# amoretti86/phylo

Measured on AMD Instinct MI355X. Metric: particle-site-likelihoods/sec, higher is better.
Workload: dtype f64; 1 GPU; primate.p N=12 S=898, GTR-init (jcmodel=false), K=2048 per GPU (K_total=2048), lambda=10, full sweep of 11 rank events; parallelism=particles sharded over 1 GPU(s), global resampling, sweeps_per_launch_set=16, contexts_in_flight=3, sweeps_in_flight=48, particles_in_flight=98304

## Files before the change

include/phylo_hip.h:

```cpp
#ifndef PHYLO_HIP_H
#define PHYLO_HIP_H

#include <stdint.h>

#ifdef __cplusplus
extern "C" {
#endif

typedef struct phylo_ctx phylo_ctx;

enum {
    PHYLO_OK = 0,
    PHYLO_EINVAL = -1,
    PHYLO_ENODEVICE = -2,
    PHYLO_EHIP = -3,
    PHYLO_ENOMEM = -4,
    PHYLO_ECOMM = -5,
    PHYLO_ESTATE = -6
};

enum {
    PHYLO_QUIRK_Q1_RAW_Q = 1u << 0,
    PHYLO_TWISTING = 1u << 1,
    PHYLO_TIME_KERNELS = 1u << 2,
// ... 91 lines not shown

int phylo_debug_stamps(phylo_ctx* ctx, uint64_t* out, int n);

int phylo_debug_reverse_lists(int N, int K, const int64_t* ancestors, const int32_t* child, int early_free, int rows_form,
                              const int32_t* lookahead_nodes, int n_lookahead, int32_t* lists, int64_t n_lists, int32_t* meta,
                              int n_meta);

int phylo_debug_lookahead_lists(int N, int K, int S, int M, const int32_t* roots_ad, int32_t* slow_flag, int32_t* image,
                                int64_t n_image, int32_t* meta, int n_meta);

int phylo_debug_reverse_plan(int N, int K, int K_local, int S, int world, int twisted, int marks, uint32_t switches, int64_t n_slow,
                             int TS, int64_t coeff_wgs, int passes_in_flight, uint32_t* mask);
int phylo_debug_sweep_plan(int N, int K, int K_local, int S, int G, int M, int world, int transport, uint32_t flags, uint32_t switches,
                           uint32_t* mask, int32_t* launches);
int phylo_debug_pack_leaf_codes(const uint8_t* codes, int N, int S, uint8_t* packed, int64_t cap, int64_t* need);
int phylo_debug_reverse_plan_batch(int N, int K, int G, int S, uint32_t switches, int64_t n_slow, int TS, int64_t coeff_wgs,
                                   int passes_in_flight, uint32_t* mask);
int phylo_debug_tree_plan(int N, int K, int G, int world, int64_t n_clades, int64_t n_topologies, int kept_whole, int64_t summary_temp,
                          int64_t branches_temp, int64_t* scalars, int64_t* summary_slab, int64_t* branches_slab, int32_t* sort_bits,
                          int32_t* launches);

int phylo_debug_device_lists(phylo_ctx* ctx, int32_t* lists, int64_t n_lists, int32_t* meta, int n_meta, int64_t* ancestors,
                             int32_t* child);
int phylo_debug_device_lists_of(phylo_ctx* ctx, const int64_t* ancestors, const int32_t* child, int32_t* lists, int64_t n_lists,
                                int32_t* meta, int n_meta);

int phylo_tree_summary(phylo_ctx* ctx, int64_t* n_clades, int32_t* n_topologies, int32_t* n_groups, phylo_stats* perf);
int phylo_tree_summary_fetch(phylo_ctx* ctx, uint64_t* clade_bits, uint64_t* clade_weight, int32_t* clade_group, uint64_t* topo_weight,
                             int32_t* topo_count, int32_t* topo_rep, int32_t* topo_group, int32_t* particle_topo, uint64_t* u, uint64_t* U);

// ... 25 lines not shown
```

phylo_amd/_ffi.py:

```python
from __future__ import annotations

import ctypes as C
import os

import numpy as np

_HERE = os.path.dirname(os.path.abspath(__file__))
LIB_PATH = os.path.join(_HERE, "csrc", "libphylo_hip.so")

PHYLO_OK = 0
QUIRK_Q1_RAW_Q = 1 << 0
TWISTING = 1 << 1
TIME_KERNELS = 1 << 2
EAGER_NODES = 1 << 3
KEEP_GRAPH = 1 << 4
ONE_LAUNCH = 1 << 5
FLAGS_DEFAULT = QUIRK_Q1_RAW_Q
COMM_ID_BYTES = 128

EXPORTS = [
    "phylo_version", "phylo_last_error", "phylo_device_count", "phylo_create", "phylo_destroy",
    "phylo_set_leaves", "phylo_set_model", "phylo_expm_batched", "phylo_cond_likelihood_K",
    "phylo_forest_loglik", "phylo_tree_loglik", "phylo_trees_loglik", "phylo_trees_loglik_rates", "phylo_debug_tree_schedule", "phylo_resample", "phylo_log_zsmc", "phylo_sweep",
    "phylo_sweep_async", "phylo_sweep_batch_async", "phylo_sweep_batch_begin", "phylo_sweep_fetch_logz", "phylo_sweep_begin", "phylo_sweep_step", "phylo_sweep_step_a", "phylo_sweep_step_group", "phylo_sweep_finish", "phylo_sweep_fetch",
    "phylo_synchronize", "phylo_sweep_node", "phylo_sweep_backward", "phylo_sweep_backward_batch",
    "phylo_tree_summary", "phylo_tree_summary_fetch", "phylo_tree_branches", "phylo_tree_branches_fetch",
    "phylo_math_probe", "phylo_debug_frechet", "phylo_debug_stamps", "phylo_debug_reverse_lists", "phylo_debug_lookahead_lists", "phylo_debug_reverse_plan", "phylo_debug_reverse_plan_batch", "phylo_debug_sweep_plan", "phylo_debug_pack_leaf_codes", "phylo_debug_tree_plan", "phylo_debug_device_lists", "phylo_debug_device_lists_of", "phylo_debug_remote_cache", "phylo_debug_site_product",
    "phylo_vi_gradients", "phylo_vi_gradients_batch", "phylo_vi_apply",
    "phylo_site_tile", "phylo_set_site_tile", "phylo_get_site_tile",
    "phylo_comm_unique_id", "phylo_comm_init", "phylo_comm_share", "phylo_comm_allgather", "phylo_comm_max", "phylo_comm_barrier",
    "phylo_comm_exchange_kind",
]


class PhyloError(RuntimeError):
    def __init__(self, code, msg):
        super().__init__("libphylo_hip error %d: %s" % (code, msg))
        self.code = code


class Stats(C.Structure):
    _fields_ = [("sweep_ms", C.c_double), ("merge_ms", C.c_double), ("merge_launches", C.c_int32),
# ... 116 lines not shown
def debug_pack_leaf_codes(codes):
    lib = load()
    cd = np.ascontiguousarray(codes, dtype=np.uint8)
    if cd.ndim != 2:
        raise ValueError("codes must be [N][S]")
    N, S = cd.shape
    need = C.c_int64(0)
    rc = lib.phylo_debug_pack_leaf_codes(_ptr(cd), C.c_int(N), C.c_int(S), None, C.c_int64(0), C.byref(need))
    if rc:
        raise PhyloError(rc, lib.phylo_last_error(None).decode())
    out = np.full(need.value, 0xff, dtype=np.uint8)
    rc = lib.phylo_debug_pack_leaf_codes(_ptr(cd), C.c_int(N), C.c_int(S), _ptr(out), C.c_int64(out.size), C.byref(need))
    if rc:
        raise PhyloError(rc, lib.phylo_last_error(None).decode())
    return out.reshape(N, -1, 64, 16)


TREE_SUMMARY_BUFS = ("u", "U", "bits", "kA", "kB", "val", "scan", "weight", "srt", "hp", "o_cbits", "o_cw", "o_tw", "child", "slot", "o_cg",
                     "o_tn", "o_trep", "o_tg", "o_ptopo", "vA", "vB", "flag", "sid", "cid", "seg_start", "count", "group", "first", "tid", "pos",
                     "err", "vC", "vD", "temp")
TREE_BRANCHES_BUFS = ("ebr", "lbr", "gbl", "gbr", "o_cs", "o_ls", "o_ts", "wA", "wB", "cpos", "kA", "kB", "vA", "vB", "cstart", "toff", "o_tc",
                      "temp")


def debug_tree_plan(N, K, G=1, world=1, n_clades=1, n_topologies=1, kept_whole=False, summary_temp=0, branches_temp=0):
    lib = load()
    ns, nb = len(TREE_SUMMARY_BUFS), len(TREE_BRANCHES_BUFS)
    sc = (C.c_int64 * 13)()
    ss, bs = (C.c_int64 * (2 * ns + 1))(), (C.c_int64 * (2 * nb + 1))()
    bits, launches = (C.c_int32 * 17)(), (C.c_int32 * 2)()
# ... 454 lines not shown

    def comm_allgather_blob(self, a):
        a = np.ascontiguousarray(a)
        world = self.K // self.K_local
        if world == 1:
            return a[None]
        out = np.empty((world,) + a.shape, dtype=a.dtype)
        self._check(self._lib.phylo_comm_allgather(self._h, _ptr(a), C.c_size_t(a.nbytes), _ptr(out)))
        return out

    def debug_remote_cache(self):
        used, cap = C.c_int(0), C.c_int(0)
        self._check(self._lib.phylo_debug_remote_cache(self._h, C.byref(used), C.byref(cap)))
        return used.value, cap.value

    def comm_exchange_kind(self):
        return ('none', 'rccl', 'hostshm', 'p2p')[int(self._lib.phylo_comm_exchange_kind(self._h))]

    def comm_max(self, value):
        v = C.c_double(float(value))
        self._check(self._lib.phylo_comm_max(self._h, C.byref(v)))
        return v.value

    def comm_barrier(self):
        self._check(self._lib.phylo_comm_barrier(self._h))


def sweep_step_group(ctxs):
    arr = (C.c_void_p * len(ctxs))(*[c._h for c in ctxs])
    rc = load().phylo_sweep_step_group(arr, C.c_int(len(ctxs)))
# ... 11 lines not shown
```

phylo_amd/csrc/phylo_hip.hip:

```cpp
#include "../../include/phylo_hip.h"

#include <cstring>
#include <hip/hip_runtime.h>
#include <hip/hip_ext.h>
#include <rocprim/device/device_radix_sort.hpp>

#include <cstdarg>
#include <cstdio>
#include <cstdlib>
#include <atomic>
#include <chrono>
#include <mutex>
#include <string>
#include <vector>

#include "phylo_comm.h"
#include "phylo_kernels.h"
#include "phylo_packed_codes.h"
#include "phylo_persist.h"
#include "phylo_grad.h"
#include "phylo_revlists_dev.h"
#include "phylo_sweep_plan.h"
#include "phylo_train.h"
#include "phylo_trees.h"
#include "phylo_trees_plan.h"
#include "phylo_treeset.h"

#include <algorithm>
#include <type_traits>

namespace {

thread_local std::string g_last_error;
// ... 12 lines not shown
    bool active = false;
    int a_done_r = -1;
    sweep_plan plan{};
};

struct env_switches {
    bool eager_nodes = false, rehearse_sharded = false, replicated_book = false, no_leaf_codes = false, one_launch = false,
         persist_stamps = false, grad_one_stream = false, grad_two_streams = false, rev_host_lists = false, no_remote_cache = false,
         no_p2p = false, grad_rows_chain = false, grad_coeff_chain = false;
    int persist_wgs = 0;
    unsigned long long p2p_wait_ticks = PK_P2P_WAIT_TICKS;
    size_t p2p_copy_words = 65536;
    int persist_nt = 256;
    int remote_cache_cap = 0;
    int scan_multi_min = 4096;
    int trees_chunk = 0;
    void read() {
        eager_nodes = getenv("PHYLO_EAGER_NODES") != nullptr;
        rehearse_sharded = getenv("PHYLO_REHEARSE_SHARDED") != nullptr;
        replicated_book = getenv("PHYLO_REPLICATED_BOOK") != nullptr;
        grad_rows_chain = getenv("PHYLO_GRAD_ROWS_CHAIN") != nullptr;
        grad_coeff_chain = getenv("PHYLO_GRAD_COEFF_CHAIN") != nullptr;
        no_leaf_codes = getenv("PHYLO_NO_LEAF_CODES") != nullptr;
        one_launch = getenv("PHYLO_ONE_LAUNCH") != nullptr;
        persist_stamps = getenv("PHYLO_PERSIST_STAMPS") != nullptr;
        grad_one_stream = getenv("PHYLO_GRAD_ONE_STREAM") != nullptr;
        grad_two_streams = getenv("PHYLO_GRAD_TWO_STREAMS") != nullptr;
        rev_host_lists = getenv("PHYLO_REV_HOST_LISTS") != nullptr;
        no_remote_cache = getenv("PHYLO_NO_REMOTE_CACHE") != nullptr;
        { const char* e = getenv("PHYLO_REMOTE_CACHE_CAP"); remote_cache_cap = e ? atoi(e) : 0; }
        { const char* e = getenv("PHYLO_SCAN_MULTI_MIN"); scan_multi_min = e ? atoi(e) : 4096; }
        { const char* e = getenv("PHYLO_TREES_CHUNK"); trees_chunk = e ? atoi(e) : 0; }
        { const char* e = getenv("PHYLO_P2P"); no_p2p = e && atoi(e) == 0; }
        { const char* e = getenv("PHYLO_P2P_COPY_WORDS"); p2p_copy_words = e ? (size_t)atol(e) : 65536; }
        { const char* e = getenv("PHYLO_P2P_WAIT_S"); p2p_wait_ticks = e && atof(e) > 0 ? (unsigned long long)(atof(e) * 1e8) : PK_P2P_WAIT_TICKS; }
        const char* w = getenv("PHYLO_PERSIST_WGS");
        persist_wgs = w ? atoi(w) : 0;
        const char* t = getenv("PHYLO_PERSIST_NT");
        persist_nt = (t && atoi(t) == 512) ? 512 : 256;
    }
};

struct phylo_ctx {
    int device = 0;
    env_switches env;
// ... 9 lines not shown
    int K = 0, N = 0, S = 0, A = 4;
    int Kloc = 0, k0 = 0;
    int rank = 0, world = 1;
    uint32_t flags = 0;
    hipStream_t stream = nullptr;
    hipEvent_t ev0 = nullptr, ev1 = nullptr;
    std::vector<hipEvent_t> kev;
    std::string err;
    bool have_leaves = false, have_model = false, swept = false, state_ready = false;
    int jc = 0;
    std::vector<double> h_lam_l, h_lam_r, h_ldf;
    double *d_Q = nullptr, *d_pi = nullptr, *d_lam_l = nullptr, *d_lam_r = nullptr, *d_ldf = nullptr;
    double* d_leaves = nullptr;
    uint8_t* d_leaf_codes = nullptr;
    uint8_t* d_leaf_packed = nullptr;
    bool leaves_coded = false;
    uint32_t* d_pair_hist = nullptr;
    bool hist_ready = false, codes_valid = false;
    double* d_pool = nullptr;
    double* d_nodell = nullptr;
    double *d_bl = nullptr, *d_br = nullptr, *d_Pmat = nullptr;
    double *d_logw = nullptr, *d_ll = nullptr;
    double* d_aux = nullptr;
    unsigned long long* d_rec = nullptr;
    int tile_override = 0;
    int site_tile = 0, ntiles = 1;
    double* d_tilev = nullptr;
    double* d_lse = nullptr;
    uint64_t* d_group_seeds = nullptr;
    char* d_tables = nullptr;
// ... 543 lines not shown
    do {
        if ((rc = bind(c)) != PHYLO_OK) break;
        {
            hipDeviceProp_t prop;
            if (hipGetDeviceProperties(&prop, dev) != hipSuccess) { rc = fail(c, PHYLO_EHIP, "hipGetDeviceProperties failed"); break; }
            c->n_cus = prop.multiProcessorCount;
        }
        if (hipStreamCreateWithFlags(&c->stream, hipStreamNonBlocking) != hipSuccess) { rc = fail(c, PHYLO_EHIP, "hipStreamCreate failed"); break; }
        if (hipEventCreate(&c->ev0) != hipSuccess || hipEventCreate(&c->ev1) != hipSuccess) { rc = fail(c, PHYLO_EHIP, "hipEventCreate failed"); break; }
        if ((rc = dalloc(c, &c->d_Q, 20 + 2 * (size_t)N)) != PHYLO_OK) break;
        c->d_pi = c->d_Q + 16;
        c->d_lam_l = c->d_Q + 20;
        c->d_lam_r = c->d_Q + 20 + N;
        if ((rc = dalloc(c, &c->d_ldf, (size_t)N + 1)) != PHYLO_OK) break;
        if ((rc = dalloc(c, &c->d_leaves, (size_t)N * S * 4)) != PHYLO_OK) break;
        if ((rc = dalloc(c, &c->d_leaf_codes, pk_codes_image_bytes(N, S))) != PHYLO_OK) break;
        c->d_leaf_packed = c->d_leaf_codes + pk_packed_offset(N, S);
        c->h_ldf.resize((size_t)N + 1);
        for (int cnt = 0; cnt <= N; ++cnt) c->h_ldf[cnt] = host_log_double_factorial(2 * (cnt > 2 ? cnt : 2) - 3);
        if (hipMemcpy(c->d_ldf, c->h_ldf.data(), ((size_t)N + 1) * 8, hipMemcpyHostToDevice) != hipSuccess) { rc = fail(c, PHYLO_EHIP, "ldf upload failed"); break; }
    } while (0);
    if (rc != PHYLO_OK) {
        g_last_error = c->err;
        phylo_destroy(c);
        return rc;
    }
    *out = c;
    return PHYLO_OK;
}

int phylo_destroy(phylo_ctx* c) {
    if (!c) return PHYLO_OK;
// ... 49 lines not shown
    HIPCHK(c, hipStreamSynchronize(c->stream));
    c->tile_override = T;
    c->site_tile = T ? T : pm_site_tile(c->S);
    c->ntiles = (c->S + c->site_tile - 1) / c->site_tile;
    free_sweep_state(c);
    c->state_ready = false;
    c->swept = false; ++c->sweep_serial;
    c->ts_done = c->tb_done = false;
    return PHYLO_OK;
}

int phylo_set_leaves(phylo_ctx* c, const double* genome) {
    CHK(bind(c));
    if (!genome) return fail(c, PHYLO_EINVAL, "genome_NxSxA is NULL");
    const size_t rows = (size_t)c->N * c->S;
    const size_t code_bytes = pk_codes_image_bytes(c->N, c->S);
    const bool pinned = rows * 32 + code_bytes <= ((size_t)8 << 20);
    std::vector<uint8_t> codes_v;
    uint8_t* codes = nullptr;
    if (pinned) {
        if (!c->h_leaves_p) {
            HIPCHK(c, hipHostMalloc((void**)&c->h_leaves_p, rows * 32 + code_bytes));
            HIPCHK(c, hipEventCreateWithFlags(&c->ev_leaves, hipEventDisableTiming));
        } else {
            HIPCHK(c, hipEventSynchronize(c->ev_leaves));
        }
        memcpy(c->h_leaves_p, genome, rows * 32);
        HIPCHK(c, hipMemcpyAsync(c->d_leaves, c->h_leaves_p, rows * 32, hipMemcpyHostToDevice, c->stream));
        codes = (uint8_t*)c->h_leaves_p + rows * 32;
    } else {
        HIPCHK(c, hipMemcpyAsync(c->d_leaves, genome, rows * 32, hipMemcpyHostToDevice, c->stream));
// ... 4 lines not shown
        bool ok = true;
        for (size_t i = 0; i < rows && ok; ++i) {
            const double* x = genome + i * 4;
            int ones = 0, zeros = 0, last = 0;
            for (int j = 0; j < 4; ++j) {
                if (pm_bits(x[j]) == pm_bits(1.0)) { ++ones; last = j; }
                else if (pm_bits(x[j]) == 0) ++zeros;
            }
            if (ones == 1 && zeros == 3) codes[i] = (uint8_t)last;
            else if (ones == 4) codes[i] = 4;
            else ok = false;
        }
        c->codes_valid = ok;
        c->leaves_coded = ok && !c->env.no_leaf_codes;
        c->hist_ready = false;
        if (ok) {
            pk_pack_leaf_codes(codes, c->N, c->S, codes + pk_packed_offset(c->N, c->S));
            HIPCHK(c, hipMemcpyAsync(c->d_leaf_codes, codes, code_bytes, hipMemcpyHostToDevice, c->stream));
        }
    }
    if (pinned) HIPCHK(c, hipEventRecord(c->ev_leaves, c->stream));
    c->have_leaves = true;
    c->last_graph = c->last_graph_twist = false;
    c->leaves_newer = true;
    CHK(refresh_leaf_ll(c));
    if (!pinned) HIPCHK(c, hipStreamSynchronize(c->stream));
    return PHYLO_OK;
}

int phylo_set_model(phylo_ctx* c, const double* Q16, const double* pi4, const double* lam_l, const double* lam_r,
                    int jc69_closed_form) {
    CHK(bind(c));
    if (!Q16 || !pi4 || !lam_l || !lam_r) return fail(c, PHYLO_EINVAL, "NULL model pointer");
// ... 664 lines not shown
    a.flag_off = c->x_flag_off[purpose];
    a.epoch = ++c->x_epoch[purpose];
    a.timeout_word = c->d_counter + 1;
    a.wait_ticks = c->env.p2p_wait_ticks;
    const size_t words = (size_t)n_arrays * count * (size_t)(c->world - 1);
    if (words > c->env.p2p_copy_words) {
        const size_t wgs = (words + 4095) / 4096;
        hipLaunchKernelGGL(pk_p2p_copy, dim3((unsigned)(wgs < 512 ? wgs : 512)), dim3(1024), 0, c->stream, a);
        CHK(launch_check(c, "pk_p2p_copy"));
        a.n_seg = 0;
    }
    hipLaunchKernelGGL(pk_p2p_exchange, dim3(1), dim3(1024), 0, c->stream, a);
    return launch_check(c, "pk_p2p_exchange");
}

static pk_rank_args rank_args(const phylo_ctx* c, int r) {
    const sweep_plan& p = c->run.plan;
    const int N = c->N, K = c->K, Kl = c->Kloc, cur = r & 1, nxt = cur ^ 1;
    const size_t plane = (size_t)K * N;
    pk_rank_args b{};
    b.r = r; b.n = N - r; b.N = N; b.S = c->S; b.K = K; b.Kloc = Kl; b.k0 = c->k0;
    b.seed = c->run.seed; b.flags = c->run.flags;
    b.Kg = p.Kg; b.group_seeds = p.G > 1 ? c->d_group_seeds : nullptr;
    b.no_store = (r == p.R - 1 && p.no_store_last) ? 1 : 0;
    if (p.graph) {
        b.roots_old = c->d_hroots + plane * r; b.cnt_old = c->d_hcnt + plane * r;
        b.roots_new = c->d_hroots + plane * (r + 1); b.cnt_new = c->d_hcnt + plane * (r + 1);
        b.rootll_old = c->d_hrootll + plane * r; b.rootll_new = c->d_hrootll + plane * (r + 1);
        b.pos_hist = c->d_pos + plane * r;
    } else {
// ... 137 lines not shown
    return launch_check(c, "pk_rank_book_packed");
}

static int step_merge(phylo_ctx* c, const pk_rank_args& b) {
    const sweep_plan& p = c->run.plan;
    const int S = c->S;
    const dim3 mgrid((unsigned)((size_t)c->Kloc * c->ntiles));
    hipEvent_t e0 = nullptr, e1 = nullptr;
    if (p.timek && !p.twist) { e0 = c->kev[2 * b.r]; e1 = c->kev[2 * b.r + 1]; }
    if (!(b.lazy || b.no_store)) {
        const size_t lds = (size_t)(c->site_tile < S ? c->site_tile : S) * 8 + 16 + PK_STORE_STAGE_BYTES;
        launch_stamped(pk_rank_merge, mgrid, dim3(PK_COLS), lds, c->stream, e0, e1, b);
    } else if (b.rec) {
        pk_pi4 pi4;
        memcpy(pi4.v, c->h_model_p + 16, sizeof pi4.v);
        launch_stamped(pk_rank_merge_nostore, mgrid, dim3(64), 0, c->stream, e0, e1, (const unsigned long long*)b.rec, b.Pmat, S, b.T,
                       b.ntiles, b.tilev, pi4);
    } else {
        launch_stamped(pk_rank_merge_nostore_ids, mgrid, dim3(64), 0, c->stream, e0, e1, b);
    }
    return launch_check(c, "pk_rank_merge");
}

static int step_tiles(phylo_ctx* c, const pk_rank_args& b) {
    hipLaunchKernelGGL(pk_tile_epilogue, dim3(cdiv(c->Kloc, 256)), dim3(256), 0, c->stream, b);
    return launch_check(c, "pk_tile_epilogue");
}

static int step_exchange(phylo_ctx* c, int r) {
    const size_t K = c->K;
    double* rows[3] = {c->d_logw + r * K, c->d_ll + r * K, c->d_nodell + c->N + r * K};
    return comm_exchange(c, rows, 3, (size_t)c->Kloc, 0);
// ... 1074 lines not shown
    const sweep_plan p = sweep_plan_form(f, k_sweep_limits);
    *mask = sweep_plan_mask(p);
    for (int r = -1; r <= p.R; ++r) launches[r + 1] = sweep_plan_launches(p, r);
    return PHYLO_OK;
}

int phylo_debug_pack_leaf_codes(const uint8_t* codes, int N, int S, uint8_t* packed, int64_t cap, int64_t* need) {
    if (N < 1 || S < 1 || !need || (packed && !codes)) return fail(nullptr, PHYLO_EINVAL, "phylo_debug_pack_leaf_codes: bad arguments");
    *need = (int64_t)pk_packed_bytes(N, S);
    if (!packed) return PHYLO_OK;
    if (cap < *need) return fail(nullptr, PHYLO_EINVAL, "phylo_debug_pack_leaf_codes: the image takes %lld bytes (got %lld)", (long long)*need, (long long)cap);
    pk_pack_leaf_codes(codes, N, S, packed);
    return PHYLO_OK;
}

int phylo_debug_tree_plan(int N, int K, int G, int world, int64_t n_clades, int64_t n_topologies, int kept_whole, int64_t summary_temp,
                          int64_t branches_temp, int64_t* scalars, int64_t* summary_slab, int64_t* branches_slab, int32_t* sort_bits,
                          int32_t* launches) {
    if (K < 1 || G < 1 || K % G != 0 || N > PK_MAX_TAXA || world < 1 || summary_temp < 0 || branches_temp < 0 || !scalars || !summary_slab ||
        !branches_slab || !sort_bits || !launches)
        return fail(nullptr, PHYLO_EINVAL, "phylo_debug_tree_plan: bad arguments");
    char why[160];
    const pt_facts f{N, K, G, world};
    if (pt_refuses(f, why, sizeof why)) return fail(nullptr, PHYLO_EINVAL, "%s", why);
    const pb_facts fb{N, K, G, world, n_clades, n_topologies, kept_whole != 0};
    if (pb_refuses(fb, why, sizeof why)) return fail(nullptr, PHYLO_ESTATE, "%s", why);
    pt_plan p = pt_plan_form(f);
    pt_plan_slab(p, (size_t)summary_temp);
    pb_plan q = pb_plan_form(fb);
    pb_plan_slab(q, (size_t)branches_temp);
// ... 643 lines not shown
```

phylo_amd/csrc/phylo_kernels.h:

```cpp
#pragma once
#include <hip/hip_runtime.h>
#include <stdint.h>

#include "phylo_math.h"
#include "phylo_packed_codes.h"

#define PK_COLS 256
#define PK_AUX 8
#define PK_MAX_TAXA 512
#define PK_MAX_GROUPS 64

enum { AUX_SUM_REM = 0, AUX_FPRIOR, AUX_LPRIOR, AUX_RPRIOR, AUX_LL_TILDE, AUX_PAREN, AUX_LOGV, AUX_Q };
#define PK_REC 16
enum { REC_BASE_L = PK_AUX, REC_BASE_R, REC_NODELL, REC_ROOTLL, REC_LL, REC_LOGW, REC_FLAGS  };
#define PK_REC_SLOTS (REC_FLAGS + 1)
static_assert(PK_REC_SLOTS <= PK_REC && PK_REC_SLOTS <= 16, "one lane per slot: with 16 lanes or more per particle the bookkeeping writes the record in one trip (pk_book_tail)");

__device__ __forceinline__ double pk_block_canon_sum(double col, double* sh4) {
#pragma unroll
    for (int off = 1; off < 64; off <<= 1) col = col + __shfl_xor(col, off, 64);
    __syncthreads();
    if ((threadIdx.x & 63) == 0) sh4[threadIdx.x >> 6] = col;
    __syncthreads();
    return ((sh4[0] + sh4[1]) + sh4[2]) + sh4[3];
// ... 1568 lines not shown
            pk_rows_pair_spec<CL, CR>(A, B, cw & 0xffu, (cw >> 8) & 0xffu, s, s1, bl, br, Pl, Pr, tabL, tabR, pi, col, flag);
            lo >>= 16;
        }
        if (m & 1) {
            if ((m >> 1) == 4) lo = hi;
            (CL ? A.cl : A.cr) = (unsigned int)lo & 0xffu;
            double xa = pk_rows_lik<CL, CR>(A, Pl, Pr, tabL, tabR, nullptr, pi);
            xa = s < s1 ? xa : 1.0;
            pm_lp_mul_spec(col, xa, flag);
        }
        if (n <= 16) break;
        n -= 16; ++Jc;
    }
    return pm_lp_flag_set(flag);
}
template <bool CL, bool CR>
__device__ __forceinline__ pm_lp pk_rows_general_v(int s0, int s1, const char* bl, const char* br, const pk_cdbl* Pc, const pk_cdbl* pik,
                                                   double (*tabL)[4], double (*tabR)[4], double* lik25) {
    const double pi[4] = {pik[0], pik[1], pik[2], pik[3]};
    double Pl[16], Pr[16];
#pragma unroll
    for (int u = 0; u < 16; ++u) {
        Pl[u] = CL ? 0.0 : Pc[u];
        Pr[u] = CR ? 0.0 : Pc[16 + u];
    }
    pk_rowregs A;
    pk_cstream c;
    pm_lp col = pm_lp_init();
    pk_cs_request<CL, CR>(c, bl, br, s0 >> 10);
    pk_rows_load_u<CL, CR>(A, bl, br, s0 + (int)(threadIdx.x & 63), s1);
    pk_rows_run_packed<CL, CR>(s0, s1, bl, br, A, c, Pl, Pr, tabL, tabR, lik25, pi, col);
    return col;
}
__device__ __forceinline__ pm_lp pk_rows_general(unsigned int fl, int s0, int s1, const char* bl, const char* br, const double* Pu,
                                                 const double* pi4, double (*tabL)[4], double (*tabR)[4], double* lik25) {
    fl = (unsigned int)__builtin_amdgcn_readfirstlane((int)fl);
    s0 = __builtin_amdgcn_readfirstlane(s0);
    s1 = __builtin_amdgcn_readfirstlane(s1);
    bl = pk_uniform_ptr(bl);
    br = pk_uniform_ptr(br);
    const pk_cdbl* Pc = (const pk_cdbl*)pk_uniform_ptr(Pu);
    const pk_cdbl* pik = (const pk_cdbl*)pk_uniform_ptr(pi4);
    if ((fl & 3u) == 3u) return pk_rows_general_v<true, true>(s0, s1, bl, br, Pc, pik, tabL, tabR, lik25);
    if (fl & 1u) return pk_rows_general_v<true, false>(s0, s1, bl, br, Pc, pik, tabL, tabR, lik25);
    return pk_rows_general_v<false, true>(s0, s1, bl, br, Pc, pik, tabL, tabR, lik25);
}
template <bool CL, bool CR>
__device__ __forceinline__ bool pk_rows_loop_rec(int s0, int s1, const char* bl, const char* br, const double* Pu, const pk_cdbl* Pc,
                                                 double (*tabL)[4], double (*tabR)[4], double* lik25, const pk_cdbl* pik, pm_lp& col) {
    const int lane = threadIdx.x & 63;
    const double pi[4] = {pik[0], pik[1], pik[2], pik[3]};
    double Pl[16], Pr[16];
#pragma unroll
    for (int u = 0; u < 16; ++u) {
        Pl[u] = CL ? 0.0 : Pc[u];
        Pr[u] = CR ? 0.0 : Pc[16 + u];
    }
    if constexpr (CL != CR) {
#pragma unroll
        for (int u = 0; u < 16; ++u) asm volatile("" : "+s"(CL ? Pr[u] : Pl[u]));
    }
    pk_rowregs A;
    pk_cstream c;
    if constexpr (CL || CR) {
// ... 16 lines not shown
        pk_wave_lds_fence();
    }
    if constexpr (CL || CR) {
        if (!redo) {
            bool flag;
            if constexpr (CL && CR) flag = pk_rows_fast_cc(s0, s1, bl, br, c, lik25, col);
            else flag = pk_rows_fast_mixed<CL, CR>(s0, s1, bl, br, A, c, Pl, Pr, tabL, tabR, pi, col);
            redo = __any(flag);
        }
        return redo;
    } else {
        pk_rows_run<CL, CR>(s0, s1, bl, br, A, Pl, Pr, tabL, tabR, lik25, pi, col);
        return false;
    }
}
struct pk_merge_kernarg { const unsigned long long* rec; const double* Pmat; int S, T, ntiles; double* tilev; pk_pi4 pi4; };
__global__ __launch_bounds__(64) __attribute__((amdgpu_waves_per_eu(7, 8), amdgpu_num_vgpr(32)))
void pk_rank_merge_nostore(const unsigned long long* __restrict__ rec, const double* __restrict__ Pmat, int S, int T, int ntiles,
                           double* __restrict__ tilev, const pk_pi4 pi4) {
    __shared__ __attribute__((aligned(16))) double tabL[PK_PAD_CODE + 1][4], tabR[PK_PAD_CODE + 1][4];
    __shared__ double lik25[PK_PAD_CODE * 6 + 1];
    const int item = (int)blockIdx.x;
    const int k = __builtin_amdgcn_readfirstlane(ntiles == 1 ? item : item / ntiles), tau = item - k * ntiles;
    const int s0 = __builtin_amdgcn_readfirstlane(tau * T), s1 = __builtin_amdgcn_readfirstlane(s0 + T < S ? s0 + T : S);
    const pk_cu64* rc = (const pk_cu64*)(rec + (size_t)k * PK_REC);
    const double* Pu = Pmat + (size_t)k * 32;
    const pk_cdbl* Pc = (const pk_cdbl*)Pu;
    PK_TOUCH4_DECL;
    PK_TOUCH4_256(Pu);
    unsigned int fl = (unsigned int)rc[REC_FLAGS];
    const char* bl = pk_uniform_ptr((const void*)rc[REC_BASE_L]);
    const char* br = pk_uniform_ptr((const void*)rc[REC_BASE_R]);
    PK_TOUCH4_END(fl);
    static_assert(offsetof(pk_merge_kernarg, pi4) == 40 && sizeof(pk_merge_kernarg) == 72, "the kernel's argument segment");
    const pk_cdbl* pi = (const pk_cdbl*)((__attribute__((address_space(4))) const char*)__builtin_amdgcn_kernarg_segment_ptr() +
                                         offsetof(pk_merge_kernarg, pi4));
    pm_lp col = pm_lp_init();
    bool redo;
    if (fl & 1u) {
        if (fl & 2u) redo = pk_rows_loop_rec<true, true>(s0, s1, bl, br, Pu, Pc, tabL, tabR, lik25, pi, col);
        else redo = pk_rows_loop_rec<true, false>(s0, s1, bl, br, Pu, Pc, tabL, tabR, lik25, pi, col);
    } else {
        if (fl & 2u) redo = pk_rows_loop_rec<false, true>(s0, s1, bl, br, Pu, Pc, tabL, tabR, lik25, pi, col);
        else redo = pk_rows_loop_rec<false, false>(s0, s1, bl, br, Pu, Pc, tabL, tabR, lik25, pi, col);
    }
    if (redo) col = pk_rows_general(fl, s0, s1, bl, br, Pu, (const double*)pi, tabL, tabR, lik25);
    const double tot = pk_wave_tree_sum(pm_lp_finish(col));
    if (threadIdx.x == 0) {
        if (ntiles != 1) {
            tilev[(size_t)k * ntiles + tau] = tot;
        } else {
            const pk_cdbl* ax = (const pk_cdbl*)rc;
            const double fl2 = ax[AUX_SUM_REM] + tot;
            const double ll = ((fl2 + ax[AUX_FPRIOR]) + ax[AUX_LPRIOR]) + ax[AUX_RPRIOR];
            const double lw = (((ll - ax[AUX_LL_TILDE]) - ax[AUX_PAREN]) + ax[AUX_LOGV]) - ax[AUX_Q];
            *(pk_gd*)rc[REC_NODELL] = tot;
            *(pk_gd*)rc[REC_ROOTLL] = tot;
            *(pk_gd*)rc[REC_LL] = ll;
            *(pk_gd*)rc[REC_LOGW] = lw;
// ... 597 lines not shown
```

Before: 611.9 billion particle-site-likelihoods/s.

## Compress alignment columns into unique site patterns for the root merge kernel

```diff
diff --git a/include/phylo_hip.h b/include/phylo_hip.h
--- a/include/phylo_hip.h
+++ b/include/phylo_hip.h
@@ -129,6 +129,10 @@
 int phylo_debug_sweep_plan(int N, int K, int K_local, int S, int G, int M, int world, int transport, uint32_t flags, uint32_t switches,
                            uint32_t* mask, int32_t* launches);
 int phylo_debug_pack_leaf_codes(const uint8_t* codes, int N, int S, uint8_t* packed, int64_t cap, int64_t* need);
+int phylo_debug_site_patterns(const uint8_t* codes, int N, int S, int32_t* U, int32_t* rep, uint16_t* image, uint32_t* rep_off,
+                              uint8_t* rep_leaf, int64_t rep_leaf_cap);
+int phylo_debug_site_patterns_rule(int S, int U, int coded, int ntiles, int sw);
+int phylo_debug_site_patterns_of(phylo_ctx* ctx, int32_t* U, int32_t* taken);
 int phylo_debug_reverse_plan_batch(int N, int K, int G, int S, uint32_t switches, int64_t n_slow, int TS, int64_t coeff_wgs,
                                    int passes_in_flight, uint32_t* mask);
 int phylo_debug_tree_plan(int N, int K, int G, int world, int64_t n_clades, int64_t n_topologies, int kept_whole, int64_t summary_temp,
diff --git a/phylo_amd/_ffi.py b/phylo_amd/_ffi.py
--- a/phylo_amd/_ffi.py
+++ b/phylo_amd/_ffi.py
@@ -25,7 +25,7 @@
     "phylo_sweep_async", "phylo_sweep_batch_async", "phylo_sweep_batch_begin", "phylo_sweep_fetch_logz", "phylo_sweep_begin", "phylo_sweep_step", "phylo_sweep_step_a", "phylo_sweep_step_group", "phylo_sweep_finish", "phylo_sweep_fetch",
     "phylo_synchronize", "phylo_sweep_node", "phylo_sweep_backward", "phylo_sweep_backward_batch",
     "phylo_tree_summary", "phylo_tree_summary_fetch", "phylo_tree_branches", "phylo_tree_branches_fetch",
-    "phylo_math_probe", "phylo_debug_frechet", "phylo_debug_stamps", "phylo_debug_reverse_lists", "phylo_debug_lookahead_lists", "phylo_debug_reverse_plan", "phylo_debug_reverse_plan_batch", "phylo_debug_sweep_plan", "phylo_debug_pack_leaf_codes", "phylo_debug_tree_plan", "phylo_debug_device_lists", "phylo_debug_device_lists_of", "phylo_debug_remote_cache", "phylo_debug_site_product",
+    "phylo_math_probe", "phylo_debug_frechet", "phylo_debug_stamps", "phylo_debug_reverse_lists", "phylo_debug_lookahead_lists", "phylo_debug_reverse_plan", "phylo_debug_reverse_plan_batch", "phylo_debug_sweep_plan", "phylo_debug_pack_leaf_codes", "phylo_debug_site_patterns", "phylo_debug_site_patterns_rule", "phylo_debug_site_patterns_of", "phylo_debug_tree_plan", "phylo_debug_device_lists", "phylo_debug_device_lists_of", "phylo_debug_remote_cache", "phylo_debug_site_product",
     "phylo_vi_gradients", "phylo_vi_gradients_batch", "phylo_vi_apply",
     "phylo_site_tile", "phylo_set_site_tile", "phylo_get_site_tile",
     "phylo_comm_unique_id", "phylo_comm_init", "phylo_comm_share", "phylo_comm_allgather", "phylo_comm_max", "phylo_comm_barrier",
@@ -172,6 +172,39 @@
     if rc:
         raise PhyloError(rc, lib.phylo_last_error(None).decode())
     return out.reshape(N, -1, 64, 16)
+
+
+SITE_PATTERN_SWITCH = {"0": 0, None: 1, "force": 2}
+
+
+def debug_site_patterns(codes):
+    lib = load()
+    cd = np.ascontiguousarray(codes, dtype=np.uint8)
+    if cd.ndim != 2:
+        raise ValueError("codes must be [N][S]")
+    N, S = cd.shape
+    nC = -(-(-(-S // 64)) // 16)
+    U = C.c_int32(0)
+    rep = np.full(S, -1, dtype=np.int32)
+    image = np.full(nC * 1024, 0xffff, dtype=np.uint16)
+    rep_off = np.full(1024, 0xffffffff, dtype=np.uint32)
+    rep_leaf = np.full(N * 1024, 0xff, dtype=np.uint8)
+    rc = lib.phylo_debug_site_patterns(_ptr(cd), C.c_int(N), C.c_int(S), C.byref(U), _ptr(rep), _ptr(image), _ptr(rep_off), _ptr(rep_leaf),
+                                       C.c_int64(rep_leaf.size))
+    if rc:
+        raise PhyloError(rc, lib.phylo_last_error(None).decode())
+    u = U.value
+    return {"U": u, "rep": rep[:u].copy(), "image": image.reshape(nC, 2, 64, 8) if u <= 8191 else None,
+            "rep_off": rep_off if u <= 512 else None,
+            "rep_leaf": rep_leaf[:N * 1024 * (-(-(-(-u // 64)) // 16))].reshape(N, -1, 64, 16) if u <= 512 else None}
+
+
+def debug_site_patterns_rule(S, U, coded=True, ntiles=1, switch=None):
+    lib = load()
+    rc = lib.phylo_debug_site_patterns_rule(C.c_int(S), C.c_int(U), C.c_int(int(coded)), C.c_int(ntiles), C.c_int(SITE_PATTERN_SWITCH[switch]))
+    if rc < 0:
+        raise PhyloError(rc, lib.phylo_last_error(None).decode())
+    return bool(rc)
 
 
 TREE_SUMMARY_BUFS = ("u", "U", "bits", "kA", "kB", "val", "scan", "weight", "srt", "hp", "o_cbits", "o_cw", "o_tw", "child", "slot", "o_cg",
@@ -656,6 +689,11 @@
         self._check(self._lib.phylo_debug_remote_cache(self._h, C.byref(used), C.byref(cap)))
         return used.value, cap.value
 
+    def debug_site_patterns(self):
+        U, taken = C.c_int32(0), C.c_int32(0)
+        self._check(self._lib.phylo_debug_site_patterns_of(self._h, C.byref(U), C.byref(taken)))
+        return U.value, bool(taken.value)
+
     def comm_exchange_kind(self):
         return ('none', 'rccl', 'hostshm', 'p2p')[int(self._lib.phylo_comm_exchange_kind(self._h))]
 
diff --git a/phylo_amd/csrc/phylo_hip.hip b/phylo_amd/csrc/phylo_hip.hip
--- a/phylo_amd/csrc/phylo_hip.hip
+++ b/phylo_amd/csrc/phylo_hip.hip
@@ -17,6 +17,7 @@
 #include "phylo_comm.h"
 #include "phylo_kernels.h"
 #include "phylo_packed_codes.h"
+#include "phylo_site_patterns.h"
 #include "phylo_persist.h"
 #include "phylo_grad.h"
 #include "phylo_revlists_dev.h"
@@ -59,6 +60,7 @@
     int persist_nt = 256;
     int remote_cache_cap = 0;
     int scan_multi_min = 4096;
+    int site_patterns = PK_PAT_AUTO;
     int trees_chunk = 0;
     void read() {
         eager_nodes = getenv("PHYLO_EAGER_NODES") != nullptr;
@@ -74,6 +76,7 @@
         rev_host_lists = getenv("PHYLO_REV_HOST_LISTS") != nullptr;
         no_remote_cache = getenv("PHYLO_NO_REMOTE_CACHE") != nullptr;
         { const char* e = getenv("PHYLO_REMOTE_CACHE_CAP"); remote_cache_cap = e ? atoi(e) : 0; }
+        { const char* e = getenv("PHYLO_SITE_PATTERNS"); site_patterns = !e ? PK_PAT_AUTO : !strcmp(e, "force") ? PK_PAT_FORCE : atoi(e) == 0 ? PK_PAT_OFF : PK_PAT_AUTO; }
         { const char* e = getenv("PHYLO_SCAN_MULTI_MIN"); scan_multi_min = e ? atoi(e) : 4096; }
         { const char* e = getenv("PHYLO_TREES_CHUNK"); trees_chunk = e ? atoi(e) : 0; }
         { const char* e = getenv("PHYLO_P2P"); no_p2p = e && atoi(e) == 0; }
@@ -113,6 +116,8 @@
     double* d_leaves = nullptr;
     uint8_t* d_leaf_codes = nullptr;
     uint8_t* d_leaf_packed = nullptr;
+    uint8_t* d_pat = nullptr;
+    int pat_U = 0;
     bool leaves_coded = false;
     uint32_t* d_pair_hist = nullptr;
     bool hist_ready = false, codes_valid = false;
@@ -686,8 +691,9 @@
         c->d_lam_r = c->d_Q + 20 + N;
         if ((rc = dalloc(c, &c->d_ldf, (size_t)N + 1)) != PHYLO_OK) break;
         if ((rc = dalloc(c, &c->d_leaves, (size_t)N * S * 4)) != PHYLO_OK) break;
-        if ((rc = dalloc(c, &c->d_leaf_codes, pk_codes_image_bytes(N, S))) != PHYLO_OK) break;
+        if ((rc = dalloc(c, &c->d_leaf_codes, pk_leaf_image_bytes(N, S))) != PHYLO_OK) break;
         c->d_leaf_packed = c->d_leaf_codes + pk_packed_offset(N, S);
+        c->d_pat = c->d_leaf_codes + pk_pat_offset(N, S);
         c->h_ldf.resize((size_t)N + 1);
         for (int cnt = 0; cnt <= N; ++cnt) c->h_ldf[cnt] = host_log_double_factorial(2 * (cnt > 2 ? cnt : 2) - 3);
         if (hipMemcpy(c->d_ldf, c->h_ldf.data(), ((size_t)N + 1) * 8, hipMemcpyHostToDevice) != hipSuccess) { rc = fail(c, PHYLO_EHIP, "ldf upload failed"); break; }
@@ -767,7 +773,7 @@
     CHK(bind(c));
     if (!genome) return fail(c, PHYLO_EINVAL, "genome_NxSxA is NULL");
     const size_t rows = (size_t)c->N * c->S;
-    const size_t code_bytes = pk_codes_image_bytes(c->N, c->S);
+    const size_t code_bytes = pk_leaf_image_bytes(c->N, c->S);
     const bool pinned = rows * 32 + code_bytes <= ((size_t)8 << 20);
     std::vector<uint8_t> codes_v;
     uint8_t* codes = nullptr;
@@ -802,9 +808,12 @@
         c->codes_valid = ok;
         c->leaves_coded = ok && !c->env.no_leaf_codes;
         c->hist_ready = false;
+        c->pat_U = 0;
         if (ok) {
             pk_pack_leaf_codes(codes, c->N, c->S, codes + pk_packed_offset(c->N, c->S));
-            HIPCHK(c, hipMemcpyAsync(c->d_leaf_codes, codes, code_bytes, hipMemcpyHostToDevice, c->stream));
+            c->pat_U = pk_pat_build(codes, c->N, c->S, codes + pk_pat_offset(c->N, c->S));
+            const size_t up_bytes = c->pat_U <= PK_PAT_MAX_U ? code_bytes : pk_codes_image_bytes(c->N, c->S);
+            HIPCHK(c, hipMemcpyAsync(c->d_leaf_codes, codes, up_bytes, hipMemcpyHostToDevice, c->stream));
         }
     }
     if (pinned) HIPCHK(c, hipEventRecord(c->ev_leaves, c->stream));
@@ -1499,6 +1508,8 @@
     return launch_check(c, "pk_p2p_exchange");
 }
 
+static bool pat_on(const phylo_ctx* c) { return pk_pat_take(c->S, c->pat_U, c->leaves_coded, c->ntiles, c->env.site_patterns); }
+
 static pk_rank_args rank_args(const phylo_ctx* c, int r) {
     const sweep_plan& p = c->run.plan;
     const int N = c->N, K = c->K, Kl = c->Kloc, cur = r & 1, nxt = cur ^ 1;
@@ -1666,8 +1677,17 @@
     } else if (b.rec) {
         pk_pi4 pi4;
         memcpy(pi4.v, c->h_model_p + 16, sizeof pi4.v);
-        launch_stamped(pk_rank_merge_nostore, mgrid, dim3(64), 0, c->stream, e0, e1, (const unsigned long long*)b.rec, b.Pmat, S, b.T,
-                       b.ntiles, b.tilev, pi4);
+        pk_pat_args pat = {nullptr, nullptr, 0, 0};
+        size_t lds = 0;
+        if (pat_on(c)) {
+            pat.pimg = (const char*)c->d_pat;
+            pat.roff = (const char*)c->d_pat + pk_pat_image_bytes(S);
+            pat.rep_delta = (long long)((c->d_pat + pk_pat_image_bytes(S) + pk_pat_rep_bytes()) - c->d_leaf_packed);
+            pat.U = c->pat_U;
+            lds = pk_pat_lds_bytes(c->pat_U);
+        }
+        launch_stamped(pk_rank_merge_nostore, mgrid, dim3(64), lds, c->stream, e0, e1, (const unsigned long long*)b.rec, b.Pmat, S, b.T,
+                       b.ntiles, b.tilev, pi4, pat);
     } else {
         launch_stamped(pk_rank_merge_nostore_ids, mgrid, dim3(64), 0, c->stream, e0, e1, b);
     }
@@ -2772,6 +2792,39 @@
     return PHYLO_OK;
 }
 
+int phylo_debug_site_patterns(const uint8_t* codes, int N, int S, int32_t* U, int32_t* rep, uint16_t* image, uint32_t* rep_off,
+                              uint8_t* rep_leaf, int64_t rep_leaf_cap) {
+    if (N < 1 || S < 1 || !codes || !U) return fail(nullptr, PHYLO_EINVAL, "phylo_debug_site_patterns: bad arguments");
+    std::vector<int32_t> pat((size_t)S), rp((size_t)S);
+    *U = pk_pat_columns(codes, N, S, pat.data(), rp.data());
+    if (rep) memcpy(rep, rp.data(), (size_t)*U * sizeof(int32_t));
+    if (image && *U <= PK_PAT_IMAGE_MAX_U) pk_pat_pack_image(pat.data(), S, *U, image);
+    if (rep_off && *U <= PK_PAT_MAX_U) pk_pat_rep_offsets(rp.data(), *U, rep_off);
+    if (rep_leaf && *U <= PK_PAT_MAX_U) {
+        if (rep_leaf_cap < (int64_t)pk_packed_bytes(N, *U))
+            return fail(nullptr, PHYLO_EINVAL, "phylo_debug_site_patterns: the representative leaf image takes %lld bytes (got %lld)",
+                        (long long)pk_packed_bytes(N, *U), (long long)rep_leaf_cap);
+        pk_pat_rep_leaf_image(codes, N, S, rp.data(), *U, rep_leaf, pk_packed_leaf_bytes(*U));
+    }
+    return PHYLO_OK;
+}
+
+int phylo_debug_site_patterns_rule(int S, int U, int coded, int ntiles, int sw) {
+    if (S < 1 || U < 0 || ntiles < 1 || sw < PK_PAT_OFF || sw > PK_PAT_FORCE) {
+        (void)fail(nullptr, PHYLO_EINVAL, "phylo_debug_site_patterns_rule: bad arguments");
+        return -1;
+    }
+    return pk_pat_take(S, U, coded != 0, ntiles, sw) ? 1 : 0;
+}
+
+int phylo_debug_site_patterns_of(phylo_ctx* c, int32_t* U, int32_t* taken) {
+    if (!c || !U || !taken) return fail(c, PHYLO_EINVAL, "phylo_debug_site_patterns_of: NULL argument");
+    if (!c->have_leaves) return fail(c, PHYLO_ESTATE, "phylo_debug_site_patterns_of needs leaves");
+    *U = c->pat_U;
+    *taken = pat_on(c) ? 1 : 0;
+    return PHYLO_OK;
+}
+
 int phylo_debug_tree_plan(int N, int K, int G, int world, int64_t n_clades, int64_t n_topologies, int kept_whole, int64_t summary_temp,
                           int64_t branches_temp, int64_t* scalars, int64_t* summary_slab, int64_t* branches_slab, int32_t* sort_bits,
                           int32_t* launches) {
diff --git a/phylo_amd/csrc/phylo_kernels.h b/phylo_amd/csrc/phylo_kernels.h
--- a/phylo_amd/csrc/phylo_kernels.h
+++ b/phylo_amd/csrc/phylo_kernels.h
@@ -4,6 +4,7 @@
 
 #include "phylo_math.h"
 #include "phylo_packed_codes.h"
+#include "phylo_site_patterns.h"
 
 #define PK_COLS 256
 #define PK_AUX 8
@@ -1606,6 +1607,95 @@
     }
     return pm_lp_flag_set(flag);
 }
+typedef __attribute__((address_space(1))) const unsigned int pk_gu32c;
+template <bool CL, bool CR>
+__device__ __forceinline__ void pk_pat_rows(pk_rowregs& x, const char* bl, const char* br, unsigned int off) {
+    if constexpr (!CL) { x.l0 = *(pk_gu4c*)(bl + off); x.l1 = *(pk_gu4c*)(bl + off + 16u); }
+    if constexpr (!CR) { x.r0 = *(pk_gu4c*)(br + off); x.r1 = *(pk_gu4c*)(br + off + 16u); }
+}
+template <bool CL, bool CR>
+__device__ __forceinline__ void pk_pat_entry(pk_rowregs& X, unsigned int code, unsigned int u, unsigned int U, const double (&Pl)[16],
+                                             const double (&Pr)[16], const double (*tabL)[4], const double (*tabR)[4],
+                                             const double (&pi)[4], double* ulik, pm_lp_flag& flag) {
+    if constexpr (CL) X.cl = code;
+    if constexpr (CR) X.cr = code;
+    double x = pk_rows_lik<CL, CR>(X, Pl, Pr, tabL, tabR, nullptr, pi);
+    x = u < U ? x : 1.0;
+    flag.f = pm_min_u32(flag.f, pm_lp_key(x));
+    ulik[u] = x;
+}
+template <bool CL, bool CR>
+__device__ __forceinline__ void pk_pat_phase1(int U, const char* bl, const char* br, const char* rl, const char* roff,
+                                              const double (&Pl)[16], const double (&Pr)[16], const double (*tabL)[4],
+                                              const double (*tabR)[4], const double (&pi)[4], double* ulik, pm_lp_flag& flag) {
+    static_assert(!(CL && CR), "an uncoded side");
+    const int nU = __builtin_amdgcn_readfirstlane((U + 63) >> 6);
+    unsigned int u = threadIdx.x & 63u;
+    unsigned long long lo = 0;
+    if constexpr (CL || CR) {
+        const pk_u4 q = *(pk_gu4c*)(rl + u * 16u);
+        lo = (unsigned long long)q.x | ((unsigned long long)q.y << 32);
+    }
+    pk_rowregs A, B;
+    unsigned int ro = *(pk_gu32c*)(roff + u * 4u);
+    pk_pat_rows<CL, CR>(A, bl, br, ro);
+    ro = *(pk_gu32c*)(roff + (u + 64u) * 4u);
+    #pragma unroll 1
+    for (int t = 0; t < (nU >> 1); ++t, u += 128u) {
+        pk_pat_rows<CL, CR>(B, bl, br, ro);
+        ro = *(pk_gu32c*)(roff + (u + 128u) * 4u);
+        const unsigned int cw = (unsigned int)lo;
+        pk_pat_entry<CL, CR>(A, cw & 0xffu, u, (unsigned int)U, Pl, Pr, tabL, tabR, pi, ulik, flag);
+        pk_pat_rows<CL, CR>(A, bl, br, ro);
+        ro = *(pk_gu32c*)(roff + (u + 192u) * 4u);
+        pk_pat_entry<CL, CR>(B, (cw >> 8) & 0xffu, u + 64u, (unsigned int)U, Pl, Pr, tabL, tabR, pi, ulik, flag);
+        lo >>= 16;
+    }
+    if (nU & 1) pk_pat_entry<CL, CR>(A, (unsigned int)lo & 0xffu, u, (unsigned int)U, Pl, Pr, tabL, tabR, pi, ulik, flag);
+    if (threadIdx.x == 0) ulik[U] = 1.0;
+}
+__device__ __forceinline__ void pk_pat_request(pk_u4& n0, pk_u4& n1, const char* pimg, int Jc) {
+    const unsigned int o = (unsigned int)Jc * (2u * PK_PAT_HALF_BYTES) + (threadIdx.x & 63u) * 16u;
+    n0 = *(pk_gu4c*)(pimg + o);
+    n1 = *(pk_gu4c*)(pimg + o + (unsigned int)PK_PAT_HALF_BYTES);
+}
+__device__ __forceinline__ void pk_pat_walk(int s1, const char* pimg, pk_u4 n0, pk_u4 n1, const double* ulik, pm_lp& col, pm_lp_flag& flag) {
+    const char* ub = (const char*)ulik;
+    int n = __builtin_amdgcn_readfirstlane((s1 + 63) >> 6), Jc = 0;
+    #pragma unroll 1
+    for (;;) {
+        const unsigned int w[8] = {n0.x, n0.y, n0.z, n0.w, n1.x, n1.y, n1.z, n1.w};
+        if (n > 16) pk_pat_request(n0, n1, pimg, Jc + 1);
+#pragma unroll
+        for (int j = 0; j < 16; j += 2) {
+            if (n < j + 2) {
+                if (n == j + 1) pm_lp_mul_normal(col, *(const double*)(ub + (w[j >> 1] & 0xffffu)));
+                break;
+            }
+            const double xa = *(const double*)(ub + (w[j >> 1] & 0xffffu));
+            const double xb = *(const double*)(ub + (w[j >> 1] >> 16));
+            pm_lp_mul2_spec_q(col, xa, xb, flag);
+        }
+        if (n <= 16) break;
+        n -= 16; ++Jc;
+    }
+}
+struct pk_pat_args { const char* pimg; const char* roff; long long rep_delta ; int U; };
+typedef __attribute__((address_space(4))) const pk_pat_args pk_pat_kargs;
+template <bool CL, bool CR>
+__device__ __forceinline__ bool pk_rows_pat(int s1, const char* bl, const char* br, const char* rl, pk_pat_kargs* pa, const double (&Pl)[16],
+                                            const double (&Pr)[16], const double (*tabL)[4], const double (*tabR)[4],
+                                            const double (&pi)[4], double* ulik, pm_lp& col) {
+    pm_lp_flag flag = pm_lp_flag_init();
+    const char* pimg = pa->pimg;
+    pk_u4 n0, n1;
+    if constexpr (CL || CR) pk_pat_request(n0, n1, pimg, 0);
+    pk_pat_phase1<CL, CR>(pa->U, bl, br, rl, pa->roff, Pl, Pr, tabL, tabR, pi, ulik, flag);
+    if constexpr (!(CL || CR)) pk_pat_request(n0, n1, pimg, 0);
+    pk_wave_lds_fence();
+    pk_pat_walk(s1, pimg, n0, n1, ulik, col, flag);
+    return pm_lp_flag_set(flag);
+}
 template <bool CL, bool CR>
 __device__ __forceinline__ pm_lp pk_rows_general_v(int s0, int s1, const char* bl, const char* br, const pk_cdbl* Pc, const pk_cdbl* pik,
                                                    double (*tabL)[4], double (*tabR)[4], double* lik25) {
@@ -1617,11 +1707,16 @@
         Pr[u] = CR ? 0.0 : Pc[16 + u];
     }
     pk_rowregs A;
-    pk_cstream c;
     pm_lp col = pm_lp_init();
-    pk_cs_request<CL, CR>(c, bl, br, s0 >> 10);
-    pk_rows_load_u<CL, CR>(A, bl, br, s0 + (int)(threadIdx.x & 63), s1);
-    pk_rows_run_packed<CL, CR>(s0, s1, bl, br, A, c, Pl, Pr, tabL, tabR, lik25, pi, col);
+    if constexpr (CL || CR) {
+        pk_cstream c;
+        pk_cs_request<CL, CR>(c, bl, br, s0 >> 10);
+        pk_rows_load_u<CL, CR>(A, bl, br, s0 + (int)(threadIdx.x & 63), s1);
+        pk_rows_run_packed<CL, CR>(s0, s1, bl, br, A, c, Pl, Pr, tabL, tabR, lik25, pi, col);
+    } else {
+        pk_rows_load<CL, CR>(A, bl, br, s0 + (int)(threadIdx.x & 63), s1);
+        pk_rows_run<CL, CR>(s0, s1, bl, br, A, Pl, Pr, tabL, tabR, lik25, pi, col);
+    }
     return col;
 }
 __device__ __forceinline__ pm_lp pk_rows_general(unsigned int fl, int s0, int s1, const char* bl, const char* br, const double* Pu,
@@ -1635,11 +1730,39 @@
     const pk_cdbl* pik = (const pk_cdbl*)pk_uniform_ptr(pi4);
     if ((fl & 3u) == 3u) return pk_rows_general_v<true, true>(s0, s1, bl, br, Pc, pik, tabL, tabR, lik25);
     if (fl & 1u) return pk_rows_general_v<true, false>(s0, s1, bl, br, Pc, pik, tabL, tabR, lik25);
-    return pk_rows_general_v<false, true>(s0, s1, bl, br, Pc, pik, tabL, tabR, lik25);
+    if (fl & 2u) return pk_rows_general_v<false, true>(s0, s1, bl, br, Pc, pik, tabL, tabR, lik25);
+    return pk_rows_general_v<false, false>(s0, s1, bl, br, Pc, pik, tabL, tabR, lik25);
+}
+template <bool CL, bool CR>
+__device__ __forceinline__ bool pk_rows_loop_pat(int s1, const char* bl, const char* br, const double* Pu, const pk_cdbl* Pc,
+                                                 double (*tabL)[4], double (*tabR)[4], const pk_cdbl* pik, pm_lp& col, pk_pat_kargs* pa,
+                                                 double* ulik) {
+    static_assert(!(CL && CR), "an uncoded side");
+    const double pi[4] = {pik[0], pik[1], pik[2], pik[3]};
+    double Pl[16], Pr[16];
+#pragma unroll
+    for (int u = 0; u < 16; ++u) {
+        Pl[u] = CL ? 0.0 : Pc[u];
+        Pr[u] = CR ? 0.0 : Pc[16 + u];
+    }
+    const char* rl = nullptr;
+    if constexpr (CL != CR) {
+#pragma unroll
+        for (int u = 0; u < 16; ++u) asm volatile("" : "+s"(CL ? Pr[u] : Pl[u]));
+        rl = (CL ? bl : br) + pa->rep_delta;
+        if constexpr (CL) pk_build_leaf_table(Pu, tabL, (int)(threadIdx.x & 63));
+        else pk_build_leaf_table(Pu + 16, tabR, (int)(threadIdx.x & 63));
+        pk_wave_lds_fence();
+    }
+    return __any(pk_rows_pat<CL, CR>(s1, bl, br, rl, pa, Pl, Pr, tabL, tabR, pi, ulik, col));
 }
 template <bool CL, bool CR>
 __device__ __forceinline__ bool pk_rows_loop_rec(int s0, int s1, const char* bl, const char* br, const double* Pu, const pk_cdbl* Pc,
-                                                 double (*tabL)[4], double (*tabR)[4], double* lik25, const pk_cdbl* pik, pm_lp& col) {
+                                                 double (*tabL)[4], double (*tabR)[4], double* lik25, const pk_cdbl* pik, pm_lp& col,
+                                                 pk_pat_kargs* pa, double* ulik) {
+    if constexpr (!(CL && CR)) {
+        if (pa->U != 0) return pk_rows_loop_pat<CL, CR>(s1, bl, br, Pu, Pc, tabL, tabR, pik, col, pa, ulik);
+    }
     const int lane = threadIdx.x & 63;
     const double pi[4] = {pik[0], pik[1], pik[2], pik[3]};
     double Pl[16], Pr[16];
@@ -1686,12 +1809,13 @@
         return false;
     }
 }
-struct pk_merge_kernarg { const unsigned long long* rec; const double* Pmat; int S, T, ntiles; double* tilev; pk_pi4 pi4; };
+struct pk_merge_kernarg { const unsigned long long* rec; const double* Pmat; int S, T, ntiles; double* tilev; pk_pi4 pi4; pk_pat_args pat; };
 __global__ __launch_bounds__(64) __attribute__((amdgpu_waves_per_eu(7, 8), amdgpu_num_vgpr(32)))
 void pk_rank_merge_nostore(const unsigned long long* __restrict__ rec, const double* __restrict__ Pmat, int S, int T, int ntiles,
-                           double* __restrict__ tilev, const pk_pi4 pi4) {
+                           double* __restrict__ tilev, const pk_pi4 pi4, const pk_pat_args pat) {
     __shared__ __attribute__((aligned(16))) double tabL[PK_PAD_CODE + 1][4], tabR[PK_PAD_CODE + 1][4];
     __shared__ double lik25[PK_PAD_CODE * 6 + 1];
+    extern __shared__ __attribute__((aligned(16))) double pk_ulik[];
     const int item = (int)blockIdx.x;
     const int k = __builtin_amdgcn_readfirstlane(ntiles == 1 ? item : item / ntiles), tau = item - k * ntiles;
     const int s0 = __builtin_amdgcn_readfirstlane(tau * T), s1 = __builtin_amdgcn_readfirstlane(s0 + T < S ? s0 + T : S);
@@ -1704,17 +1828,20 @@
     const char* bl = pk_uniform_ptr((const void*)rc[REC_BASE_L]);
     const char* br = pk_uniform_ptr((const void*)rc[REC_BASE_R]);
     PK_TOUCH4_END(fl);
-    static_assert(offsetof(pk_merge_kernarg, pi4) == 40 && sizeof(pk_merge_kernarg) == 72, "the kernel's argument segment");
+    static_assert(offsetof(pk_merge_kernarg, pi4) == 40 && offsetof(pk_merge_kernarg, pat) == 72 && sizeof(pk_merge_kernarg) == 104,
+                  "the kernel's argument segment");
+    pk_pat_kargs* pa = (pk_pat_kargs*)((__attribute__((address_space(4))) const char*)__builtin_amdgcn_kernarg_segment_ptr() +
+                                       offsetof(pk_merge_kernarg, pat));
     const pk_cdbl* pi = (const pk_cdbl*)((__attribute__((address_space(4))) const char*)__builtin_amdgcn_kernarg_segment_ptr() +
                                          offsetof(pk_merge_kernarg, pi4));
     pm_lp col = pm_lp_init();
     bool redo;
     if (fl & 1u) {
-        if (fl & 2u) redo = pk_rows_loop_rec<true, true>(s0, s1, bl, br, Pu, Pc, tabL, tabR, lik25, pi, col);
-        else redo = pk_rows_loop_rec<true, false>(s0, s1, bl, br, Pu, Pc, tabL, tabR, lik25, pi, col);
+        if (fl & 2u) redo = pk_rows_loop_rec<true, true>(s0, s1, bl, br, Pu, Pc, tabL, tabR, lik25, pi, col, pa, pk_ulik);
+        else redo = pk_rows_loop_rec<true, false>(s0, s1, bl, br, Pu, Pc, tabL, tabR, lik25, pi, col, pa, pk_ulik);
     } else {
-        if (fl & 2u) redo = pk_rows_loop_rec<false, true>(s0, s1, bl, br, Pu, Pc, tabL, tabR, lik25, pi, col);
-        else redo = pk_rows_loop_rec<false, false>(s0, s1, bl, br, Pu, Pc, tabL, tabR, lik25, pi, col);
+        if (fl & 2u) redo = pk_rows_loop_rec<false, true>(s0, s1, bl, br, Pu, Pc, tabL, tabR, lik25, pi, col, pa, pk_ulik);
+        else redo = pk_rows_loop_rec<false, false>(s0, s1, bl, br, Pu, Pc, tabL, tabR, lik25, pi, col, pa, pk_ulik);
     }
     if (redo) col = pk_rows_general(fl, s0, s1, bl, br, Pu, (const double*)pi, tabL, tabR, lik25);
     const double tot = pk_wave_tree_sum(pm_lp_finish(col));
diff --git a/phylo_amd/csrc/phylo_site_patterns.h b/phylo_amd/csrc/phylo_site_patterns.h
--- /dev/null
+++ b/phylo_amd/csrc/phylo_site_patterns.h
@@ -0,0 +1,103 @@
+#pragma once
+#include <stddef.h>
+#include <stdint.h>
+#include <string.h>
+
+#include <vector>
+
+#include "phylo_packed_codes.h"
+
+#define PK_PAT_MAX_U 512
+#define PK_PAT_REP_WORDS 1024
+#define PK_PAT_HALF_BYTES 1024
+#define PK_PAT_IMAGE_MAX_U 8191
+
+enum { PK_PAT_OFF = 0, PK_PAT_AUTO = 1, PK_PAT_FORCE = 2 };
+
+static inline size_t pk_pat_image_bytes(int S) { return (size_t)pk_packed_chunks(S) * 2 * PK_PAT_HALF_BYTES; }
+static inline size_t pk_pat_rep_bytes() { return (size_t)PK_PAT_REP_WORDS * 4; }
+static inline size_t pk_pat_offset(int N, int S) { return (pk_codes_image_bytes(N, S) + 15) & ~(size_t)15; }
+static inline size_t pk_pat_rep_offset(int N, int S) { return pk_pat_offset(N, S) + pk_pat_image_bytes(S); }
+static inline size_t pk_pat_leaf_offset(int N, int S) { return pk_pat_rep_offset(N, S) + pk_pat_rep_bytes(); }
+static inline size_t pk_leaf_image_bytes(int N, int S) { return pk_pat_leaf_offset(N, S) + pk_packed_bytes(N, S); }
+static inline size_t pk_pat_lds_bytes(int U) { return ((size_t)((U + 63) / 64) * 64 + 1) * 8; }
+
+static inline int pk_pat_columns(const uint8_t* codes, int N, int S, int32_t* pat, int32_t* rep) {
+    std::vector<uint64_t> h((size_t)S, 0xcbf29ce484222325ull);
+    for (int leaf = 0; leaf < N; ++leaf) {
+        const uint8_t* row = codes + (size_t)leaf * S;
+        for (int s = 0; s < S; ++s) h[s] = (h[s] ^ row[s]) * 0x100000001b3ull;
+    }
+    size_t cap = 16;
+    while (cap < (size_t)S * 2) cap <<= 1;
+    std::vector<int32_t> slot(cap, -1);
+    int U = 0;
+    for (int s = 0; s < S; ++s) {
+        uint64_t x = h[s];
+        x ^= x >> 29;
+        size_t i = (size_t)(x * 0x9e3779b97f4a7c15ull >> 20) & (cap - 1);
+        int u = -1;
+        for (;; i = (i + 1) & (cap - 1)) {
+            const int32_t cand = slot[i];
+            if (cand < 0) break;
+            const int r = rep[cand];
+            if (h[r] != h[s]) continue;
+            bool eq = true;
+            for (int leaf = 0; leaf < N && eq; ++leaf) eq = codes[(size_t)leaf * S + r] == codes[(size_t)leaf * S + s];
+            if (eq) { u = cand; break; }
+        }
+        if (u < 0) {
+            u = U++;
+            rep[u] = s;
+            slot[i] = u;
+        }
+        pat[s] = u;
+    }
+    return U;
+}
+static inline void pk_pat_pack_image(const int32_t* pat, int S, int U, uint16_t* image) {
+    const size_t n = pk_pat_image_bytes(S) / 2;
+    const uint16_t pad = (uint16_t)(8 * U);
+    for (size_t i = 0; i < n; ++i) image[i] = pad;
+    const int nsteps = (S + 63) / 64;
+    for (int q = 0; q < nsteps; ++q) {
+        const int cnt = S - 64 * q < 64 ? S - 64 * q : 64;
+        uint16_t* d = image + ((size_t)(q / PK_CHUNK_STEPS) * 2 + (q % PK_CHUNK_STEPS) / 8) * (PK_PAT_HALF_BYTES / 2) + q % 8;
+        const int32_t* p = pat + (size_t)64 * q;
+        for (int c = 0; c < cnt; ++c) d[c * 8] = (uint16_t)(8 * p[c]);
+    }
+}
+static inline void pk_pat_rep_offsets(const int32_t* rep, int U, uint32_t* off) {
+    for (int u = 0; u < PK_PAT_REP_WORDS; ++u) off[u] = u < U ? 32u * (uint32_t)rep[u] : 0u;
+}
+static inline void pk_pat_rep_leaf_image(const uint8_t* codes, int N, int S, const int32_t* rep, int U, uint8_t* packed, size_t stride) {
+    std::vector<uint8_t> cu((size_t)U);
+    for (int leaf = 0; leaf < N; ++leaf) {
+        for (int u = 0; u < U; ++u) cu[u] = codes[(size_t)leaf * S + rep[u]];
+        pk_pack_leaf_codes(cu.data(), 1, U, packed + (size_t)leaf * stride);
+    }
+}
+static inline int pk_pat_build(const uint8_t* codes, int N, int S, uint8_t* tables) {
+    std::vector<int32_t> pat((size_t)S), rep((size_t)S);
+    const int U = pk_pat_columns(codes, N, S, pat.data(), rep.data());
+    if (U <= PK_PAT_MAX_U) {
+        pk_pat_pack_image(pat.data(), S, U, (uint16_t*)tables);
+        pk_pat_rep_offsets(rep.data(), U, (uint32_t*)(tables + pk_pat_image_bytes(S)));
+        pk_pat_rep_leaf_image(codes, N, S, rep.data(), U, tables + pk_pat_image_bytes(S) + pk_pat_rep_bytes(), pk_packed_leaf_bytes(S));
+    }
+    return U;
+}
+
+#define PK_PAT_C_STEP 38
+#define PK_PAT_C_PHASE1 33
+#define PK_PAT_C_WALK 7
+#define PK_PAT_C_FIXED 30
+static inline bool pk_pat_valid(int S, int U, bool coded, int ntiles) {
+    return coded && ntiles == 1 && S >= 1 && U >= 1 && U <= PK_PAT_MAX_U;
+}
+static inline bool pk_pat_take(int S, int U, bool coded, int ntiles, int sw) {
+    if (sw == PK_PAT_OFF || !pk_pat_valid(S, U, coded, ntiles)) return false;
+    if (sw == PK_PAT_FORCE) return true;
+    const long nS = (S + 63) / 64, nU = (U + 63) / 64;
+    return 10 * (nU * PK_PAT_C_PHASE1 + nS * PK_PAT_C_WALK + PK_PAT_C_FIXED) <= 8 * nS * PK_PAT_C_STEP;
+}
```

Result: faster. 670.3 billion particle-site-likelihoods/s (median of 6 runs) (+9.5%).
